# GabrielGao0310/SVT-av1_pro-anchor-v2.1.0-

Measured on AMD Instinct MI355X. Metric: CDEF+restoration+SAD Mpixels/s on 4K10b, higher is better.
Workload: dtype u16

## Files before the change

include/svtgpu.h:

```cpp
#ifndef SVTGPU_H
#define SVTGPU_H

#include <stdbool.h>
#include <stddef.h>
#include <stdint.h>

#ifdef __cplusplus
extern "C" {
#endif

#define SVTGPU_OK 0
#define SVTGPU_ERR_INVALID_ARG (-1)
#define SVTGPU_ERR_HIP (-2)
#define SVTGPU_ERR_UNSUPPORTED (-3)
#define SVTGPU_ERR_NO_DEVICE (-4)
#define SVTGPU_ERR_OOM (-5)

#define SVTGPU_BLOCK_4X4 0
#define SVTGPU_BLOCK_4X8 1
#define SVTGPU_BLOCK_8X4 2
#define SVTGPU_BLOCK_8X8 3

typedef struct SvtGpuCdefList {
    uint8_t by;
// ... 21 lines not shown
} SvtGpuConvolveParams;

#ifndef SVTGPU_CDEF_LIST_T
#define SVTGPU_CDEF_LIST_T SvtGpuCdefList
#endif
#ifndef SVTGPU_BLOCK_SIZE_T
#define SVTGPU_BLOCK_SIZE_T int32_t
#endif
#ifndef SVTGPU_SGR_PARAMS_T
#define SVTGPU_SGR_PARAMS_T SvtGpuSgrParams
#endif
#ifndef SVTGPU_CONVOLVE_PARAMS_T
#define SVTGPU_CONVOLVE_PARAMS_T SvtGpuConvolveParams
#endif
#ifndef SVTGPU_BIT_DEPTH_T
#define SVTGPU_BIT_DEPTH_T int32_t
#endif
#ifndef SVTGPU_ERROR_T
#define SVTGPU_ERROR_T uint32_t
#endif

int         svtgpu_device_available(void);
const char *svtgpu_version(void);
#define SVTGPU_ABI_VERSION 14
int32_t     svtgpu_abi_version(void);
const char *svtgpu_error_string(int code);

typedef struct SvtGpuContext SvtGpuContext;
int   svtgpu_context_create(int device, SvtGpuContext **out);
void  svtgpu_context_destroy(SvtGpuContext *ctx);
void *svtgpu_context_stream(SvtGpuContext *ctx);
int   svtgpu_synchronize(SvtGpuContext *ctx, void *stream);
int  svtgpu_stream_create(SvtGpuContext *ctx, int32_t priority, void **out_stream);
void svtgpu_stream_destroy(void *stream);
int  svtgpu_buffer_alloc(SvtGpuContext *ctx, size_t bytes, void **dev_out);
void svtgpu_buffer_free(void *dev);
int  svtgpu_buffer_upload(void *dev, const void *host, size_t bytes, void *stream);
int  svtgpu_buffer_download(void *host, const void *dev, size_t bytes, void *stream);

typedef struct SvtGpuFrame SvtGpuFrame;
int      svtgpu_frame_create(SvtGpuContext *ctx, int32_t width, int32_t height, int32_t bit_depth,
                             SvtGpuFrame **out);
void     svtgpu_frame_destroy(SvtGpuFrame *f);
int32_t  svtgpu_frame_stride(const SvtGpuFrame *f, int plane);
void    *svtgpu_frame_plane_ptr(SvtGpuFrame *f, int plane);
int svtgpu_frame_upload(SvtGpuFrame *f, int plane, const void *host, int32_t host_stride, void *stream);
int svtgpu_frame_download(const SvtGpuFrame *f, int plane, void *host, int32_t host_stride, void *stream);
// ... 725 lines not shown
int  svtgpu_lr_set_units(SvtGpuLrState *s, int32_t plane, const SvtGpuRestUnit *units, void *stream);
int  svtgpu_lr_apply_frame(SvtGpuLrState *s, const SvtGpuFrame *deblocked, const SvtGpuFrame *cdef_out,
                           SvtGpuFrame *out, const int32_t frame_type[3], void *stream);


typedef struct SvtGpuLrSearchControls {
    int32_t wn_enabled, wn_use_chroma, wn_filter_tap_lvl, wn_use_refinement, wn_max_one_refinement_step;
    int32_t sg_enabled, sg_use_chroma;
    int32_t sg_start_ep[2], sg_end_ep[2], sg_ep_inc[2], sg_refine[2];
    int32_t rdmult;
    int32_t switchable_restore_cost[3], wiener_restore_cost[2], sgrproj_restore_cost[2];
} SvtGpuLrSearchControls;
typedef struct SvtGpuLrUnitSearch {
    int64_t        sse[3];
    SvtGpuRestUnit wiener, sgrproj;
} SvtGpuLrUnitSearch;
int svtgpu_lr_search_frame(SvtGpuLrState *s, const SvtGpuFrame *recon, const SvtGpuFrame *source,
                           const SvtGpuLrSearchControls *ctrls, int32_t frame_type_out[3],
                           SvtGpuLrUnitSearch *const search_out[3], void *stream);
int svtgpu_lr_search_frame_async(SvtGpuLrState *s, const SvtGpuFrame *recon, const SvtGpuFrame *source,
                                 const SvtGpuLrSearchControls *ctrls, void *stream);
int svtgpu_lr_read_result(SvtGpuLrState *s, int32_t frame_type_out[3], void *stream);
int svtgpu_lr_read_units(SvtGpuLrState *s, int32_t plane, SvtGpuRestUnit *units_out, void *stream);
int svtgpu_lr_search_units(SvtGpuLrState *s, const SvtGpuFrame *recon, const SvtGpuFrame *source,
                           const SvtGpuLrSearchControls *ctrls, const int32_t row_begin[3], const int32_t row_end[3],
                           SvtGpuLrUnitSearch *const search_out[3], void *stream);
int svtgpu_lr_finish_plane(const SvtGpuLrSearchControls *ctrls, int32_t plane, int32_t nunits,
                           const SvtGpuLrUnitSearch *records, int32_t *frame_type_out, SvtGpuRestUnit *units_out);
int svtgpu_lr_finish_frame(const SvtGpuLrSearchControls *ctrls, const int32_t nunits[3],
                           const SvtGpuLrUnitSearch *const records[3], int32_t frame_type_out[3],
                           SvtGpuRestUnit *const units_out[3]);
int svtgpu_lr_set_tile(SvtGpuLrState *s, const int32_t units[3][4], const int32_t out[3][4], SvtGpuComm *comm);
typedef struct SvtGpuLrProfile {
    int32_t launches[6];
    float   ms[6];
    double  bytes[6];
    int32_t searches;
    float   ms_events[6];
} SvtGpuLrProfile;
int svtgpu_lr_profile(SvtGpuLrState *s, int32_t enable, SvtGpuLrProfile *totals);
int svtgpu_transfer_bytes(uint64_t *h2d, uint64_t *d2h, int32_t reset);
int svtgpu_lr_controls_for_level(int32_t wn_level, int32_t sg_level, SvtGpuLrSearchControls *c);

#define SVTGPU_CCSO_PAD 5
#define SVTGPU_CCSO_LUT 2048
typedef struct SvtGpuCcsoParams {
// ... 46 lines not shown
```

svt-av1_pro-anchor-v2.1.0-_amd/csrc/lr_common.h:

```cpp
#pragma once
#include "svtgpu_internal.h"

#include <vector>

struct SvtGpuLrState {
    SvtGpuContext  *ctx;
    int32_t         width, height;
    int32_t         unit_size[3], hunits[3], vunits[3];
    SvtGpuRestUnit *d_units[3];
    int16_t        *d_flt;
    size_t          flt_bytes;
    void           *d_work;
    size_t          work_bytes;
    void           *h_pin;
    size_t          pin_bytes;
    void           *prof;
    void                *plan_work;
    std::vector<uint8_t> plan_bytes;
    hipEvent_t           pin_free;
    hipStream_t          wst;
    hipEvent_t           ev_fork, ev_join;
    void                *d_qarena;
    size_t               qarena_bytes;
    void                *d_sxarena;
    size_t               sxarena_bytes;
    uint32_t             sx_epoch;
    int32_t              tile_units[3][4], tile_out[3][4];
    SvtGpuComm          *comm;
    int32_t             *h_fout, *h_fout_dev;
    int32_t              fin_seq, fin_pending;
    int32_t              last_ft[3];
};
void lr_profiler_destroy(void *prof);
int  lr_make_wiener_stream(SvtGpuLrState *s);
inline int lr_plane_w(const SvtGpuLrState *s, int p) { return p ? (s->width + 1) >> 1 : s->width; }
inline int lr_plane_h(const SvtGpuLrState *s, int p) { return p ? (s->height + 1) >> 1 : s->height; }
inline bool lr_frame_fits(const SvtGpuLrState *s, const SvtGpuFrame *f) {
    return f && f->width == ((s->width + 7) & ~7) && f->height == ((s->height + 7) & ~7);
}

namespace {

constexpr int NTHR = 256;
__constant__ int c_sgr_r[16][2] = {{2, 1}, {2, 1}, {2, 1}, {2, 1}, {2, 1}, {2, 1}, {2, 1}, {2, 1},
                                   {2, 1}, {2, 1}, {0, 1}, {0, 1}, {0, 1}, {0, 1}, {2, 0}, {2, 0}};
__constant__ int c_sgr_s[16][2] = {{140, 3236}, {112, 2158}, {93, 1618}, {80, 1438}, {70, 1295}, {58, 1177},
                                   {47, 1079},  {37, 996},   {30, 925},  {25, 863},  {-1, 2589}, {-1, 1618},
                                   {-1, 1177},  {-1, 925},   {56, -1},   {22, -1}};
__constant__ int c_x_by_xplus1[256] = {
    1,   128, 171, 192, 205, 213, 219, 224, 228, 230, 233, 235, 236, 238, 239, 240, 241, 242, 243, 243, 244, 244,
    245, 245, 246, 246, 247, 247, 247, 247, 248, 248, 248, 248, 249, 249, 249, 249, 249, 250, 250, 250, 250, 250,
    250, 250, 251, 251, 251, 251, 251, 251, 251, 251, 251, 251, 252, 252, 252, 252, 252, 252, 252, 252, 252, 252,
    252, 252, 252, 252, 252, 252, 252, 253, 253, 253, 253, 253, 253, 253, 253, 253, 253, 253, 253, 253, 253, 253,
    253, 253, 253, 253, 253, 253, 253, 253, 253, 253, 253, 253, 253, 253, 254, 254, 254, 254, 254, 254, 254, 254,
// ... 92 lines not shown
```

svt-av1_pro-anchor-v2.1.0-_amd/csrc/lr_search.hip:

```cpp
#include <algorithm>
#include <chrono>
#include <climits>
#include <cstdio>
#include <cstdlib>
#include <cmath>
#include <cstring>
#include <type_traits>
#include <vector>

#include "lr_common.h"


namespace {

struct Tile {
    int32_t plane, unit, x0, y0, w, h;
};
struct URect {
    int32_t h_start, h_end, v_start, v_end;
};
constexpr int PRJ_MIN0 = -96, PRJ_MAX0 = 31, PRJ_MIN1 = -32, PRJ_MAX1 = 95;
const int     kHostSgrR[16][2] = {{2, 1}, {2, 1}, {2, 1}, {2, 1}, {2, 1}, {2, 1}, {2, 1}, {2, 1},
                              {2, 1}, {2, 1}, {0, 1}, {0, 1}, {0, 1}, {0, 1}, {2, 0}, {2, 0}};
const int     kHostSgrS1[16] = {3236, 2158, 1618, 1438, 1295, 1177, 1079, 996, 925, 863, 2589, 1618, 1177, 925, -1, -1};

struct PlaneArgs {
    const void *dgd, *src;
    int16_t    *flt;
    int16_t    *dxp;
    int32_t     dstride, sstride, W, H, bd, fstride;
    int32_t     unit_base, pair_base, ne;
    int32_t     eps[16];
    int32_t     f1e[16];
    int32_t     win, nval;
    int64_t     mh_off;
};
struct SearchArgs {
    PlaneArgs      pl[3];
    const Tile    *tiles;
    const URect   *units;
    const int32_t *tile0;
};

template <typename T>
__device__ inline int px(const T *p, int stride, int W, int H, int y, int x) {
    y = min(max(y, 0), H - 1);
    x = min(max(x, 0), W - 1);
    return p[(size_t)y * stride + x];
}

__device__ inline unsigned long long wave_sum(unsigned long long v) { return wave_sum_lane63(v); }
constexpr int WAVE_LAST = 63;

constexpr int PROF_NL = 512, PROF_SP = 64;
#define PROF_BEGIN(tk)                                                                                      \
    if ((tk) && threadIdx.x == 0)                                                                           \
// ... 233 lines not shown
        }
    }
    __syncthreads();
    long long *dst = part + (size_t)tl * NVAL;
    for (int k = tid; k < NVAL; k += 256) dst[k] = out[k];
    PROF_END(tk);
}

__global__ void reduce_parts_kernel(const long long *part, const int32_t *unit_tile0, int tile_begin, int nvals,
                                    long long *out, unsigned long long *tk) {
    PROF_BEGIN(tk);
    const int u = blockIdx.x, t0 = unit_tile0[u] - tile_begin, t1 = unit_tile0[u + 1] - tile_begin;
    for (int k = blockIdx.y * blockDim.x + threadIdx.x; k < nvals; k += gridDim.y * blockDim.x) {
        long long s = 0;
        for (int t = t0; t < t1; t++) s += part[(size_t)t * nvals + k];
        out[(size_t)u * nvals + k] = s;
    }
    PROF_END(tk);
}


constexpr int SG_V = 70, SG_B = 66, SG_NT = 1024, SG_NQ = (SG_B * SG_B + SG_NT - 1) / SG_NT;
constexpr int SG_NQ2 = ((SG_B + 1) / 2 * SG_B + SG_NT - 1) / SG_NT;

__device__ inline uint32_t sgr_z(int sum, int sq, int n, int s, int sh) {
    const uint32_t a = (uint32_t)((sq + ((1 << (2 * sh)) >> 1)) >> (2 * sh));
    const uint32_t b = (uint32_t)((sum + ((1 << sh) >> 1)) >> sh);
    const uint32_t an = __umul24(a, (uint32_t)n), bb = __umul24(b, b);
    const uint32_t p  = an < bb ? 0u : an - bb;
    return min((p * (uint32_t)s + (1u << 19)) >> 20, 255u);
}
__device__ inline int sgr_ab_pack(int A, int sum, int n) {
    const int B = (int)((__umul24(__umul24((uint32_t)(256 - A), (uint32_t)sum), (uint32_t)c_one_by_x[n - 1]) + (1u << 11)) >> 12);
    return (B << 9) | A;
}

template <typename T>
__global__ __launch_bounds__(SG_NT) void sgr_flt_kernel(const SearchArgs A, unsigned long long *tk) {
    PROF_BEGIN(tk);
    __shared__ int ab1[2][SG_B * SG_B], ab2[2][SG_B * SG_B];
    __shared__ int      xby[256];
    static_assert(SG_V * SG_V * 2 <= SG_B * SG_B * 4, "tile image fits the aliased map buffer");
    uint16_t *const v = (uint16_t *)ab1[1];
    const Tile       t = A.tiles[xcd_swizzle(blockIdx.x, gridDim.x)];
    const PlaneArgs &P = A.pl[t.plane];
    const T         *d = (const T *)P.dgd;
    for (int i = threadIdx.x; i < (t.h + 6) * (t.w + 6); i += SG_NT) {
        const int r = i / (t.w + 6), c = i % (t.w + 6);
        v[r * SG_V + c] = (uint16_t)px(d, P.dstride, P.W, P.H, t.y0 + r - 3, t.x0 + c - 3);
    }
    if (threadIdx.x < 256) xby[threadIdx.x] = c_x_by_xplus1[threadIdx.x];
    __syncthreads();
    const uint16_t *v0 = v + 3 * SG_V + 3;
    auto lds_pair = [&](int a) {
        const uint32_t *w = (const uint32_t *)v + (a >> 1);
        return __builtin_amdgcn_alignbit(w[1], w[0], (a & 1) * 16);
    };
    const int       bw = t.w + 2, nq = (t.h + 2) * bw, nq2 = (t.h + 3) / 2 * bw;
    int s1[SG_NQ], q1[SG_NQ], s2[SG_NQ2], q2[SG_NQ2], m2q[SG_NQ2];
#pragma unroll
    for (int k = 0; k < SG_NQ; k++) {
        const int q = threadIdx.x + k * SG_NT;
        s1[k] = q1[k] = 0;
        if (q < nq) {
            const int y = q / bw - 1, x = q % bw - 1;
#pragma unroll
            for (int dy = -1; dy <= 1; dy++) {
                const int      a  = (y + dy + 3) * SG_V + x + 3;
                const uint32_t pr = lds_pair(a - 1);
                const int      p[3] = {(int)(pr & 0xFFFF), (int)(pr >> 16), (int)v[a + 1]};
#pragma unroll
                for (int j = 0; j < 3; j++) s1[k] += p[j], q1[k] += p[j] * p[j];
            }
        }
    }
#pragma unroll
    for (int k = 0; k < SG_NQ2; k++) {
        const int i = threadIdx.x + k * SG_NT, row = i / bw, x = i - row * bw - 1, y = 2 * row - 1;
        s2[k] = q2[k] = 0;
        m2q[k] = i < nq2 ? (y + 1) * bw + x + 1 : -1;
        if (i < nq2) {
#pragma unroll
            for (int dy = -2; dy <= 2; dy++) {
                const int      a  = (y + dy + 3) * SG_V + x + 3;
                const uint32_t pa = lds_pair(a - 2), pb = lds_pair(a);
                const int      p[5] = {(int)(pa & 0xFFFF), (int)(pa >> 16), (int)(pb & 0xFFFF), (int)(pb >> 16), (int)v[a + 2]};
#pragma unroll
                for (int j = 0; j < 5; j++) s2[k] += p[j], q2[k] += p[j] * p[j];
            }
        }
    }
    const int fr = (int)threadIdx.x / t.w, fx = (int)threadIdx.x - fr * t.w, fy0 = 4 * fr;
    const bool fon = fy0 < t.h;
    int        pix[4];
#pragma unroll
    for (int k = 0; k < 4; k++) pix[k] = fon && fy0 + k < t.h ? v0[(fy0 + k) * SG_V + fx] : 0;
    const int   fq  = fx + 1;
    const size_t fo = (size_t)(t.y0 + fy0) * P.fstride + t.x0 + fx;
    const size_t pn = (size_t)P.fstride * P.H;
    const int sh = P.bd - 8;
    auto build_ab = [&](int e) {
        const int ep = P.eps[e], r0 = c_sgr_r[ep][0], r1 = c_sgr_r[ep][1];
        int      *m1 = ab1[e & 1], *m2 = ab2[e & 1];
        if (r1 && P.f1e[e] == e) {
            const int sp = c_sgr_s[ep][1];
            uint32_t  z[SG_NQ];
            int       a[SG_NQ];
#pragma unroll
            for (int k = 0; k < SG_NQ; k++) z[k] = sgr_z(s1[k], q1[k], 9, sp, sh);
#pragma unroll
            for (int k = 0; k < SG_NQ; k++) a[k] = xby[z[k]];
#pragma unroll
            for (int k = 0; k < SG_NQ; k++) {
                const int q = threadIdx.x + k * SG_NT;
                if (q < nq) m1[q] = sgr_ab_pack(a[k], s1[k], 9);
            }
        }
        if (r0) {
            const int sp = c_sgr_s[ep][0];
            uint32_t  z[SG_NQ2];
            int       a[SG_NQ2];
#pragma unroll
            for (int k = 0; k < SG_NQ2; k++) z[k] = sgr_z(s2[k], q2[k], 25, sp, sh);
#pragma unroll
            for (int k = 0; k < SG_NQ2; k++) a[k] = xby[z[k]];
#pragma unroll
            for (int k = 0; k < SG_NQ2; k++)
                if (m2q[k] >= 0) m2[m2q[k]] = sgr_ab_pack(a[k], s2[k], 25);
        }
    };
    build_ab(0);
    __syncthreads();
    for (int e = 0; e < P.ne; e++) {
        if (e + 1 < P.ne) build_ab(e + 1);
        const int  ep = P.eps[e], r0 = c_sgr_r[ep][0], r1 = c_sgr_r[ep][1];
        const int *ab1e = ab1[e & 1], *ab2e = ab2[e & 1];
        int16_t  *f0g = P.flt + (size_t)e * 2 * pn, *f1g = f0g + pn;
        if (fon) {
            struct Row { int s, sa, c, ca; };
            auto row = [&](const int *M, int ry) {
                const int *Q = M + (min(ry, t.h) + 1) * bw + fq;
                const int  l = Q[-1], c = Q[0], r = Q[1];
                Row        w;
                w.c = c, w.ca = c & 511, w.s = l + c + r, w.sa = (l & 511) + w.ca + (r & 511);
                return w;
            };
            const int nk = min(4, t.h - fy0);
            if (r0) {
                Row up = row(ab2e, fy0 - 1);
#pragma unroll
                for (int h = 0; h < 2; h++) {
                    const int k = 2 * h;
                    if (k >= nk) break;
                    const Row dn = row(ab2e, fy0 + k + 1);
                    {
                        const int c6 = up.c + dn.c, a6 = up.ca + dn.ca;
                        const int c5 = up.s - up.c + dn.s - dn.c, a5 = up.sa - up.ca + dn.sa - dn.ca;
                        const int aa = a6 * 6 + a5 * 5, bb = ((c6 - a6) >> 9) * 6 + ((c5 - a5) >> 9) * 5;
                        f0g[fo + (size_t)k * P.fstride] =
                            (int16_t)((((int)__umul24((uint32_t)aa, (uint32_t)pix[k]) + bb + (1 << 8)) >> 9) - (pix[k] << 4));
                    }
                    if (k + 1 < nk) {
                        const int a6 = dn.ca, a5 = dn.sa - dn.ca;
                        const int aa = a6 * 6 + a5 * 5, bb = ((dn.c - a6) >> 9) * 6 + ((dn.s - dn.c - a5) >> 9) * 5;
                        f0g[fo + (size_t)(k + 1) * P.fstride] =
                            (int16_t)((((int)__umul24((uint32_t)aa, (uint32_t)pix[k + 1]) + bb + (1 << 7)) >> 8) -
                                      (pix[k + 1] << 4));
                    }
                    up = dn;
                }
            }
            if (r1 && P.f1e[e] == e) {
                Row pv = row(ab1e, fy0 - 1), cu = row(ab1e, fy0);
#pragma unroll
                for (int k = 0; k < 4; k++) {
                    if (k >= nk) break;
                    const Row nx = row(ab1e, fy0 + k + 1);
                    const int c4 = cu.s + pv.c + nx.c, a4 = cu.sa + pv.ca + nx.ca;
                    const int c3 = pv.s - pv.c + nx.s - nx.c, a3 = pv.sa - pv.ca + nx.sa - nx.ca;
                    const int aa = a4 * 4 + a3 * 3, bb = ((c4 - a4) >> 9) * 4 + ((c3 - a3) >> 9) * 3;
                    f1g[fo + (size_t)k * P.fstride] =
                        (int16_t)((((int)__umul24((uint32_t)aa, (uint32_t)pix[k]) + bb + (1 << 8)) >> 9) - (pix[k] << 4));
                    pv = cu, cu = nx;
                }
            }
        }
        __syncthreads();
    }
    PROF_END(tk);
}

typedef short v2i16s __attribute__((ext_vector_type(2)));
__device__ inline uint32_t pk_sub16(uint32_t a, uint32_t b) {
    return __builtin_bit_cast(uint32_t, __builtin_bit_cast(v2i16s, a) - __builtin_bit_cast(v2i16s, b));
}

template <typename T>
__global__ __launch_bounds__(256) void sgr_sse_kernel(const SearchArgs A, const int32_t *best, unsigned long long *err,
                                                      unsigned long long *tk) {
    PROF_BEGIN(tk);
    const Tile       t = A.tiles[xcd_swizzle(blockIdx.x, gridDim.x)];
    const PlaneArgs &P = A.pl[t.plane];
    const int       *b = best + t.unit * 4;
    const int        e = b[0], ep = b[1], xq0 = b[2], xq1 = b[3], r0 = c_sgr_r[ep][0], r1 = c_sgr_r[ep][1];
    const T         *d = (const T *)P.dgd, *s = (const T *)P.src;
    const size_t     pn = (size_t)P.fstride * P.H;
    const int16_t   *f0 = P.flt + (size_t)e * 2 * pn, *f1 = P.flt + (size_t)(e >= 0 ? P.f1e[e] : e) * 2 * pn + pn;
// ... 2233 lines not shown
        HIP_TRY(hipMalloc(&s->d_flt, 2 * flt_elems));
        s->flt_bytes = 2 * flt_elems;
    }
    uint8_t *wb = (uint8_t *)s->d_work, *hb = (uint8_t *)s->h_pin;
    auto     dp = [&](size_t o) { return (void *)(wb + o); };
    auto     hp = [&](size_t o) { return (void *)(hb + o); };
    SearchArgs A;
    std::memset(&A, 0, sizeof A);
    size_t flt_off = 0;
    for (int p = 0; p < nplanes; p++) {
        PlaneArgs &P = A.pl[p];
        P.dgd = rec->plane[p], P.src = src->plane[p], P.dstride = rec->stride[p], P.sstride = src->stride[p];
        P.W = lr_plane_w(s, p), P.H = lr_plane_h(s, p), P.bd = rec->bit_depth, P.fstride = (P.W + 63) & ~63;
        P.flt       = s->d_flt + flt_off;
        P.unit_base = pp[p].unit_base, P.pair_base = pp[p].pair_base, P.ne = pp[p].ne;
        for (int k = 0; k < pp[p].ne; k++) {
            P.eps[k] = pp[p].eps[k], P.f1e[k] = k;
            for (int j = 0; j < k; j++)
                if (kHostSgrR[P.eps[k]][1] && kHostSgrS1[P.eps[j]] == kHostSgrS1[P.eps[k]]) {
                    P.f1e[k] = j;
                    break;
                }
        }
        P.win = pp[p].win, P.nval = pp[p].nval, P.mh_off = (int64_t)pp[p].mh_off;
        P.dxp = pp[p].sg ? P.flt + (size_t)pp[p].ne * 2 * P.fstride * P.H : nullptr;
        if (pp[p].sg) flt_off += (size_t)(pp[p].ne * 2 + 1) * P.fstride * P.H;
    }
    A.tiles = (const Tile *)dp(o_tiles), A.units = (const URect *)dp(o_units), A.tile0 = (const int32_t *)dp(o_t0);
    auto *d_t0 = (int32_t *)dp(o_t0);
    LrProfiler         *prof = (LrProfiler *)s->prof;
    unsigned long long *pc   = prof ? prof->d_px : nullptr;
    auto run = [&](int c, hipStream_t ls, auto &&launch) {
        const int ev = prof ? prof->ev_begin(c, ls) : -1;
        launch(prof ? prof->slot(c) : nullptr);
        if (prof) prof->ev_end(ev, ls);
    };
    if (prof) prof->start();
    {
        uint8_t *pl = (uint8_t *)hp(h_plan);
        std::memset(pl, 0, plan_span);
        std::memcpy(pl + o_tiles, tiles.data(), sizeof(Tile) * nt_all);
        std::memcpy(pl + o_units, units.data(), sizeof(URect) * n_all);
        std::memcpy(pl + o_t0, tile0.data(), 4 * (n_all + 1));
        std::memcpy(pl + o_witem, wr_items.data(), sizeof(WrItem) * (size_t)n_wr);
        std::memcpy(pl + o_sritem, sr_items.data(), sizeof(SrItem) * (size_t)n_sr);
        std::memcpy(pl + o_dst, dst.data(), 4 * (size_t)n_all);
        if (s->plan_work != s->d_work || s->plan_bytes.size() != plan_span ||
            std::memcmp(s->plan_bytes.data(), pl, plan_span)) {
            HIP_TRY(hipMemcpyAsync(dp(0), pl, plan_span, hipMemcpyHostToDevice, st));
// ... 561 lines not shown
    }
    int32_t rb[3], re[3], cb[3], ce[3];
    for (int p = 0; p < 3; p++)
        cb[p] = s->tile_units[p][0], rb[p] = s->tile_units[p][1], ce[p] = s->tile_units[p][2], re[p] = s->tile_units[p][3];
    if (!svtgpu_comm_tiled(s->comm))
        for (int p = 0; p < 3; p++) rb[p] = cb[p] = 0, re[p] = s->vunits[p], ce[p] = s->hunits[p];
    return recon->bytes_per_sample == 2
        ? search_frame<uint16_t>(s, recon, source, ctrls, nplanes, rb, re, cb, ce, nullptr, nullptr, st, 1)
        : search_frame<uint8_t>(s, recon, source, ctrls, nplanes, rb, re, cb, ce, nullptr, nullptr, st, 1);
}

extern "C" int svtgpu_lr_read_units(SvtGpuLrState *s, int32_t plane, SvtGpuRestUnit *units_out, void *stream) {
    if (!s || plane < 0 || plane > 2 || !units_out) return SVTGPU_ERR_INVALID_ARG;
    hipStream_t st = pick_stream(s->ctx, stream);
    if (s->fin_pending)
        if (int rc = lr_collect(s, st, nullptr)) return rc;
    const size_t n = (size_t)s->hunits[plane] * s->vunits[plane];
    HIP_TRY(hipMemcpyAsync(units_out, s->d_units[plane], sizeof(SvtGpuRestUnit) * n, hipMemcpyDeviceToHost, st));
    svtgpu_count_xfer(1, sizeof(SvtGpuRestUnit) * n);
    HIP_TRY(hipStreamSynchronize(st));
    return SVTGPU_OK;
}

extern "C" int svtgpu_lr_read_result(SvtGpuLrState *s, int32_t frame_type_out[3], void *stream) {
    if (!s || !frame_type_out) return SVTGPU_ERR_INVALID_ARG;
    if (s->fin_pending) return lr_collect(s, pick_stream(s->ctx, stream), frame_type_out);
    for (int p = 0; p < 3; p++) frame_type_out[p] = s->last_ft[p];
    return SVTGPU_OK;
}
```

svt-av1_pro-anchor-v2.1.0-_amd/svtgpu.py:

```python
import ctypes
import os

import numpy as np

_HERE = os.path.dirname(os.path.abspath(__file__))
LIB_PATH = os.environ.get("SVTGPU_LIB") or os.path.join(_HERE, "lib", "libsvtgpu.so")
HEADER_PATH = os.path.join(os.path.dirname(_HERE), "include", "svtgpu.h")

SVTGPU_OK = 0
TOTAL_STRENGTHS = 64
MAX_STRENGTHS = 16


class CdefList(ctypes.Structure):
    _fields_ = [("by", ctypes.c_uint8), ("bx", ctypes.c_uint8)]


class CdefControls(ctypes.Structure):
    _fields_ = [
        ("first_pass_fs_num", ctypes.c_uint8),
        ("default_second_pass_fs_num", ctypes.c_uint8),
        ("default_first_pass_fs", ctypes.c_uint8 * TOTAL_STRENGTHS),
        ("default_second_pass_fs", ctypes.c_uint8 * TOTAL_STRENGTHS),
        ("default_first_pass_fs_uv", ctypes.c_int8 * TOTAL_STRENGTHS),
# ... 481 lines not shown
    "svtgpu_md_out_device_ptr": (_P, [_P]),
    "svtgpu_md_moments_device_ptr": (_P, [_P]),
    "svtgpu_md_expand": (ctypes.c_int, [_P, _I32, _I32, _P]),
    "svtgpu_md_layout": (None, [_P, _P, _P]),
    "svtgpu_av1_wiener_convolve_add_src": (None, [_P, ctypes.c_ssize_t, _P, ctypes.c_ssize_t, _P, _P, _I32, _I32,
                                                  ctypes.POINTER(ConvolveParams)]),
    "svtgpu_av1_highbd_wiener_convolve_add_src": (None, [_P, ctypes.c_ssize_t, _P, ctypes.c_ssize_t, _P, _P, _I32,
                                                         _I32, ctypes.POINTER(ConvolveParams), _I32]),
    "svtgpu_av1_selfguided_restoration": (None, [_P, _I32, _I32, _I32, _P, _P, _I32, _I32, _I32, _I32]),
    "svtgpu_apply_selfguided_restoration": (None, [_P, _I32, _I32, _I32, _I32, _P, _P, _I32, _P, _I32, _I32]),
    "svtgpu_lr_state_create": (ctypes.c_int, [_P, _I32, _I32, _P, ctypes.POINTER(_P)]),
    "svtgpu_lr_state_destroy": (None, [_P]),
    "svtgpu_lr_units": (ctypes.c_int, [_P, _I32, ctypes.POINTER(_I32), ctypes.POINTER(_I32)]),
    "svtgpu_lr_set_units": (ctypes.c_int, [_P, _I32, _P, _P]),
    "svtgpu_lr_apply_frame": (ctypes.c_int, [_P, _P, _P, _P, _P, _P]),
    "svtgpu_lr_search_frame": (ctypes.c_int, [_P, _P, _P, ctypes.POINTER(LrSearchControls), _P, _P, _P]),
    "svtgpu_lr_controls_for_level": (ctypes.c_int, [_I32, _I32, ctypes.POINTER(LrSearchControls)]),
    "svtgpu_lr_search_units": (ctypes.c_int, [_P, _P, _P, ctypes.POINTER(LrSearchControls), _P, _P, _P, _P]),
    "svtgpu_lr_finish_plane": (ctypes.c_int, [ctypes.POINTER(LrSearchControls), _I32, _I32, _P, _P, _P]),
    "svtgpu_lr_finish_frame": (ctypes.c_int, [ctypes.POINTER(LrSearchControls), _P, _P, _P, _P]),
    "svtgpu_lr_search_frame_async": (ctypes.c_int, [_P, _P, _P, ctypes.POINTER(LrSearchControls), _P]),
    "svtgpu_lr_read_result": (ctypes.c_int, [_P, _P, _P]),
    "svtgpu_lr_read_units": (ctypes.c_int, [_P, _I32, _P, _P]),
    "svtgpu_lr_profile": (ctypes.c_int, [_P, _I32, _P]),
    "svtgpu_transfer_bytes": (ctypes.c_int, [_P, _P, _I32]),
    "svtgpu_comm_unique_id": (ctypes.c_int, [_P]),
    "svtgpu_comm_create": (ctypes.c_int, [_P, _I32, _I32, _P, ctypes.POINTER(_P)]),
    "svtgpu_comm_create_bounded": (ctypes.c_int, [_P, _I32, _I32, _P, _I32, _I32, ctypes.POINTER(_P)]),
    "svtgpu_comm_create_host": (ctypes.c_int, [_I32, _I32, _P, ctypes.POINTER(_P)]),
    "svtgpu_comm_destroy": (None, [_P]),
    "svtgpu_comm_nranks": (_I32, [_P]),
    "svtgpu_comm_rank": (_I32, [_P]),
    "svtgpu_comm_allreduce_u64": (ctypes.c_int, [_P, _P, ctypes.c_size_t, _I32, _P]),
    "svtgpu_comm_set_timeout": (ctypes.c_int, [_P, _I32]),
    "svtgpu_comm_timeout_ms": (_I32, [_P]),
    "svtgpu_comm_set_slot": (ctypes.c_int, [_P, _I32]),
    "svtgpu_comm_failed": (_I32, [_P]),
    "svtgpu_comm_sync": (ctypes.c_int, [_P, _P]),
    "svtgpu_debug_stall": (ctypes.c_int, [_P, _P, _I32]),
    "svtgpu_shim_calls": (ctypes.c_uint64, []),
    "svtgpu_tile_plan": (ctypes.c_int, [_I32, _I32, _P, _I32, _I32, _I32, _P]),
    "svtgpu_tile_plan_sb": (ctypes.c_int, [_I32, _I32, _P, _I32, _I32, _I32, _I32, _P]),
    "svtgpu_tile_plan_crop": (ctypes.c_int, [_I32, _I32, _I32, _I32, _P, _I32, _I32, _I32, _I32, _P]),
    "svtgpu_dlf_set_tile": (ctypes.c_int, [_P, _P, _P, _P]),
    "svtgpu_dlf_set_crop": (ctypes.c_int, [_P, ctypes.c_int32, ctypes.c_int32]),
    "svtgpu_cdef_set_tile": (ctypes.c_int, [_P, _P, _P, _P]),
# ... 598 lines not shown
            check(lib().svtgpu_lr_units(h, p, ctypes.byref(hu), ctypes.byref(vu)))
            self.units.append((hu.value, vu.value))

    def set_units(self, plane, units, stream=None):
        u = np.ascontiguousarray(units, REST_UNIT_DTYPE)
        assert len(u) == self.units[plane][0] * self.units[plane][1], (len(u), self.units[plane])
        check(lib().svtgpu_lr_set_units(self.h, plane, ptr(u), stream))

    def search(self, recon, source, ctrls, stream=None, records=False):
        ft = np.zeros(3, np.int32)
        recs = [np.zeros(hu * vu, LR_UNIT_SEARCH_DTYPE) for hu, vu in self.units] if records else None
        rp = (ctypes.c_void_p * 3)(*[r.ctypes.data for r in recs]) if records else None
        check(lib().svtgpu_lr_search_frame(self.h, recon.h, source.h, ctypes.byref(ctrls), ptr(ft), rp, stream))
        return ([int(x) for x in ft], recs) if records else [int(x) for x in ft]

    def search_async(self, recon, source, ctrls, stream=None):
        check(lib().svtgpu_lr_search_frame_async(self.h, recon.h, source.h, ctypes.byref(ctrls), stream))

    def read_units(self, plane, stream=None):
        u = np.zeros(self.units[plane][0] * self.units[plane][1], REST_UNIT_DTYPE)
        check(lib().svtgpu_lr_read_units(self.h, plane, ptr(u), stream))
        return u

    def read_result(self, stream=None):
        ft = np.zeros(3, np.int32)
        check(lib().svtgpu_lr_read_result(self.h, ptr(ft), stream))
        return [int(x) for x in ft]

    def search_units(self, recon, source, ctrls, row_begin, row_end, records=None, stream=None):
        if records is None:
            records = [np.zeros(hu * vu, LR_UNIT_SEARCH_DTYPE) for hu, vu in self.units]
        rb = np.ascontiguousarray(row_begin, np.int32)
        re_ = np.ascontiguousarray(row_end, np.int32)
        rp = (ctypes.c_void_p * 3)(*[r.ctypes.data for r in records])
        check(lib().svtgpu_lr_search_units(self.h, recon.h, source.h, ctypes.byref(ctrls), ptr(rb), ptr(re_), rp,
                                           stream))
        return records

    PROFILE_CLASSES = ("stats", "sgr_filters", "wiener_trials", "projection", "other", "sgr_moments")

    def profile(self, enable=True, events=False, serial=False):
        if enable is True:
            mask = -1
        elif not enable:
            mask = 0
        else:
# ... 11 lines not shown
        out["searches"] = int(raw["searches"][0])
        return out

    def set_tile(self, units=None, out=None, comm=None):
        check(lib().svtgpu_lr_set_tile(self.h, _rects3(units), _rects3(out), comm.h if comm else None))

    def apply(self, deblocked, cdef_out, out, frame_type, stream=None):
        ft = None if frame_type is None else np.ascontiguousarray(frame_type, np.int32)
        check(lib().svtgpu_lr_apply_frame(self.h, deblocked.h, cdef_out.h, out.h, None if ft is None else ptr(ft),
                                          stream))

    def close(self):
        if self.h:
            lib().svtgpu_lr_state_destroy(self.h)
            self.h = None

    def __del__(self):
        try:
            self.close()
        except Exception:
            pass


def lr_controls(wn_level, sg_level, rdmult=0, switchable=(0, 0, 0), wiener=(0, 0), sgrproj=(0, 0)):
    c = LrSearchControls()
    check(lib().svtgpu_lr_controls_for_level(wn_level, sg_level, ctypes.byref(c)))
    c.rdmult = rdmult
    for i, v in enumerate(switchable):
        c.switchable_restore_cost[i] = v
    for i, v in enumerate(wiener):
        c.wiener_restore_cost[i] = v
    for i, v in enumerate(sgrproj):
        c.sgrproj_restore_cost[i] = v
    return c


def lr_finish_plane(ctrls, plane, records):
    r = np.ascontiguousarray(records, LR_UNIT_SEARCH_DTYPE)
    units = np.zeros(len(r), REST_UNIT_DTYPE)
    ft = _I32()
    check(lib().svtgpu_lr_finish_plane(ctypes.byref(ctrls), plane, len(r), ptr(r), ctypes.byref(ft), ptr(units)))
    return ft.value, units


def lr_finish_frame(ctrls, records):
    rs = [np.ascontiguousarray(r, LR_UNIT_SEARCH_DTYPE) for r in records]
# ... 260 lines not shown
```

Baseline: 3547.

## Restructure SGR filter kernel: precompute variance terms, repack A/B maps, 2x2 output per thread

The self-guided filter search kernel now turns the box sums into variance terms once, before the eps loop, and pre-multiplies sums by the one_by_x constants. The strength values per eps are resolved on the host, so the hot loop no longer does constant-memory radius/strength lookups. The A/B map packing is reformulated to store 256-A with an 11-bit field so each output pixel needs fewer ops. Each thread now produces a 2x2 pixel block with paired 32-bit stores instead of a 4-row column, and a waves-per-EU hint is added. A debug readback API for the SGR filter planes is also added, which slightly enlarges the state struct and bumps the ABI version.

```diff
diff --git a/include/svtgpu.h b/include/svtgpu.h
--- a/include/svtgpu.h
+++ b/include/svtgpu.h
@@ -67,7 +67,7 @@
 
 int         svtgpu_device_available(void);
 const char *svtgpu_version(void);
-#define SVTGPU_ABI_VERSION 14
+#define SVTGPU_ABI_VERSION 15
 int32_t     svtgpu_abi_version(void);
 const char *svtgpu_error_string(int code);
 
@@ -839,6 +839,8 @@
                                  const SvtGpuLrSearchControls *ctrls, void *stream);
 int svtgpu_lr_read_result(SvtGpuLrState *s, int32_t frame_type_out[3], void *stream);
 int svtgpu_lr_read_units(SvtGpuLrState *s, int32_t plane, SvtGpuRestUnit *units_out, void *stream);
+int svtgpu_lr_read_sgr_planes(SvtGpuLrState *s, int32_t plane, int32_t slot, int32_t *ep_out, int16_t *flt0,
+                              int16_t *flt1, void *stream);
 int svtgpu_lr_search_units(SvtGpuLrState *s, const SvtGpuFrame *recon, const SvtGpuFrame *source,
                            const SvtGpuLrSearchControls *ctrls, const int32_t row_begin[3], const int32_t row_end[3],
                            SvtGpuLrUnitSearch *const search_out[3], void *stream);
diff --git a/svt-av1_pro-anchor-v2.1.0-_amd/csrc/lr_common.h b/svt-av1_pro-anchor-v2.1.0-_amd/csrc/lr_common.h
--- a/svt-av1_pro-anchor-v2.1.0-_amd/csrc/lr_common.h
+++ b/svt-av1_pro-anchor-v2.1.0-_amd/csrc/lr_common.h
@@ -30,6 +30,8 @@
     int32_t             *h_fout, *h_fout_dev;
     int32_t              fin_seq, fin_pending;
     int32_t              last_ft[3];
+    int16_t             *sg_flt[3];
+    int32_t              sg_fstride[3], sg_w[3], sg_h[3], sg_ne[3], sg_eps[3][16], sg_f1e[3][16];
 };
 void lr_profiler_destroy(void *prof);
 int  lr_make_wiener_stream(SvtGpuLrState *s);
diff --git a/svt-av1_pro-anchor-v2.1.0-_amd/csrc/lr_search.hip b/svt-av1_pro-anchor-v2.1.0-_amd/csrc/lr_search.hip
--- a/svt-av1_pro-anchor-v2.1.0-_amd/csrc/lr_search.hip
+++ b/svt-av1_pro-anchor-v2.1.0-_amd/csrc/lr_search.hip
@@ -23,6 +23,7 @@
 const int     kHostSgrR[16][2] = {{2, 1}, {2, 1}, {2, 1}, {2, 1}, {2, 1}, {2, 1}, {2, 1}, {2, 1},
                               {2, 1}, {2, 1}, {0, 1}, {0, 1}, {0, 1}, {0, 1}, {2, 0}, {2, 0}};
 const int     kHostSgrS1[16] = {3236, 2158, 1618, 1438, 1295, 1177, 1079, 996, 925, 863, 2589, 1618, 1177, 925, -1, -1};
+const int     kHostSgrS0[16] = {140, 112, 93, 80, 70, 58, 47, 37, 30, 25, -1, -1, -1, -1, 56, 22};
 
 struct PlaneArgs {
     const void *dgd, *src;
@@ -32,6 +33,7 @@
     int32_t     unit_base, pair_base, ne;
     int32_t     eps[16];
     int32_t     f1e[16];
+    int32_t     es0[16], es1[16];
     int32_t     win, nval;
     int64_t     mh_off;
 };
@@ -311,24 +313,33 @@
 
 constexpr int SG_V = 70, SG_B = 66, SG_NT = 1024, SG_NQ = (SG_B * SG_B + SG_NT - 1) / SG_NT;
 constexpr int SG_NQ2 = ((SG_B + 1) / 2 * SG_B + SG_NT - 1) / SG_NT;
-
-__device__ inline uint32_t sgr_z(int sum, int sq, int n, int s, int sh) {
+constexpr int      SG_AB = 11;
+constexpr uint32_t SG_AM = (1u << SG_AB) - 1;
+
+__device__ inline uint32_t sgr_p(int sum, int sq, int n, int sh) {
     const uint32_t a = (uint32_t)((sq + ((1 << (2 * sh)) >> 1)) >> (2 * sh));
     const uint32_t b = (uint32_t)((sum + ((1 << sh) >> 1)) >> sh);
     const uint32_t an = __umul24(a, (uint32_t)n), bb = __umul24(b, b);
-    const uint32_t p  = an < bb ? 0u : an - bb;
-    return min((p * (uint32_t)s + (1u << 19)) >> 20, 255u);
-}
-__device__ inline int sgr_ab_pack(int A, int sum, int n) {
-    const int B = (int)((__umul24(__umul24((uint32_t)(256 - A), (uint32_t)sum), (uint32_t)c_one_by_x[n - 1]) + (1u << 11)) >> 12);
-    return (B << 9) | A;
+    return an < bb ? 0u : an - bb;
+}
+__device__ inline uint32_t sgr_z(uint32_t p, int s) { return min((p * (uint32_t)s + (1u << 19)) >> 20, 255u); }
+__device__ inline int sgr_ab_pack(int Am, uint32_t so) {
+    const uint32_t x = __umul24((uint32_t)Am, so) + (1u << 11);
+    return (int)(((x >> 1) & ~SG_AM) | (uint32_t)Am);
+}
+template <int WA, int WB, int SH>
+__device__ inline int sgr_pixel(uint32_t ca, uint32_t cb, int npix) {
+    const int ma = __mul24((int)(ca & SG_AM), npix) + (int)(ca >> SG_AB);
+    const int mb = __mul24((int)(cb & SG_AM), npix) + (int)(cb >> SG_AB);
+    return (__mul24(ma, WA) + (__mul24(mb, WB) + (1 << (SH - 1)))) >> SH;
 }
 
 template <typename T>
-__global__ __launch_bounds__(SG_NT) void sgr_flt_kernel(const SearchArgs A, unsigned long long *tk) {
+__global__ __launch_bounds__(SG_NT) __attribute__((amdgpu_waves_per_eu(8))) void sgr_flt_kernel(const SearchArgs A,
+                                                                                                unsigned long long *tk) {
     PROF_BEGIN(tk);
     __shared__ int ab1[2][SG_B * SG_B], ab2[2][SG_B * SG_B];
-    __shared__ int      xby[256];
+    __shared__ int xby[256];
     static_assert(SG_V * SG_V * 2 <= SG_B * SG_B * 4, "tile image fits the aliased map buffer");
     uint16_t *const v = (uint16_t *)ab1[1];
     const Tile       t = A.tiles[xcd_swizzle(blockIdx.x, gridDim.x)];
@@ -338,7 +349,7 @@
         const int r = i / (t.w + 6), c = i % (t.w + 6);
         v[r * SG_V + c] = (uint16_t)px(d, P.dstride, P.W, P.H, t.y0 + r - 3, t.x0 + c - 3);
     }
-    if (threadIdx.x < 256) xby[threadIdx.x] = c_x_by_xplus1[threadIdx.x];
+    if (threadIdx.x < 256) xby[threadIdx.x] = 256 - c_x_by_xplus1[threadIdx.x];
     __syncthreads();
     const uint16_t *v0 = v + 3 * SG_V + 3;
     auto lds_pair = [&](int a) {
@@ -347,6 +358,7 @@
     };
     const int       bw = t.w + 2, nq = (t.h + 2) * bw, nq2 = (t.h + 3) / 2 * bw;
     int s1[SG_NQ], q1[SG_NQ], s2[SG_NQ2], q2[SG_NQ2], m2q[SG_NQ2];
+    const int sh = P.bd - 8;
 #pragma unroll
     for (int k = 0; k < SG_NQ; k++) {
         const int q = threadIdx.x + k * SG_NT;
@@ -362,6 +374,7 @@
                 for (int j = 0; j < 3; j++) s1[k] += p[j], q1[k] += p[j] * p[j];
             }
         }
+        q1[k] = (int)sgr_p(s1[k], q1[k], 9, sh), s1[k] = (int)__umul24((uint32_t)s1[k], 455u);
     }
 #pragma unroll
     for (int k = 0; k < SG_NQ2; k++) {
@@ -378,100 +391,96 @@
                 for (int j = 0; j < 5; j++) s2[k] += p[j], q2[k] += p[j] * p[j];
             }
         }
-    }
-    const int fr = (int)threadIdx.x / t.w, fx = (int)threadIdx.x - fr * t.w, fy0 = 4 * fr;
-    const bool fon = fy0 < t.h;
-    int        pix[4];
-#pragma unroll
-    for (int k = 0; k < 4; k++) pix[k] = fon && fy0 + k < t.h ? v0[(fy0 + k) * SG_V + fx] : 0;
-    const int   fq  = fx + 1;
-    const size_t fo = (size_t)(t.y0 + fy0) * P.fstride + t.x0 + fx;
-    const size_t pn = (size_t)P.fstride * P.H;
-    const int sh = P.bd - 8;
+        q2[k] = (int)sgr_p(s2[k], q2[k], 25, sh), s2[k] = (int)__umul24((uint32_t)s2[k], 164u);
+    }
+    const int  cpn = (t.w + 1) >> 1, fr = (int)threadIdx.x / cpn;
+    const bool fon = 2 * fr < t.h;
+    const int  fx = fon ? 2 * ((int)threadIdx.x - fr * cpn) : 0, fy0 = fon ? 2 * fr : 0;
+    const bool row1 = fy0 + 1 < t.h, col1 = fx + 1 < t.w;
+    int        npix[2][2];
+#pragma unroll
+    for (int j = 0; j < 2; j++)
+#pragma unroll
+        for (int i = 0; i < 2; i++) npix[j][i] = -(int)v0[(fy0 + j) * SG_V + fx + i];
+    int mrow[4];
+#pragma unroll
+    for (int j = 0; j < 4; j++) mrow[j] = (min(fy0 - 1 + j, t.h) + 1) * bw + fx;
+    const uint32_t fob = 2u * ((uint32_t)(t.y0 + fy0) * (uint32_t)P.fstride + (uint32_t)(t.x0 + fx));
+    const size_t   pn  = (size_t)P.fstride * P.H;
     auto build_ab = [&](int e) {
-        const int ep = P.eps[e], r0 = c_sgr_r[ep][0], r1 = c_sgr_r[ep][1];
+        const int sp0 = P.es0[e], sp1 = P.es1[e];
         int      *m1 = ab1[e & 1], *m2 = ab2[e & 1];
-        if (r1 && P.f1e[e] == e) {
-            const int sp = c_sgr_s[ep][1];
-            uint32_t  z[SG_NQ];
-            int       a[SG_NQ];
-#pragma unroll
-            for (int k = 0; k < SG_NQ; k++) z[k] = sgr_z(s1[k], q1[k], 9, sp, sh);
+        if (sp1) {
+            uint32_t z[SG_NQ];
+            int      a[SG_NQ];
+#pragma unroll
+            for (int k = 0; k < SG_NQ; k++) z[k] = sgr_z((uint32_t)q1[k], sp1);
 #pragma unroll
             for (int k = 0; k < SG_NQ; k++) a[k] = xby[z[k]];
 #pragma unroll
             for (int k = 0; k < SG_NQ; k++) {
                 const int q = threadIdx.x + k * SG_NT;
-                if (q < nq) m1[q] = sgr_ab_pack(a[k], s1[k], 9);
-            }
-        }
-        if (r0) {
-            const int sp = c_sgr_s[ep][0];
-            uint32_t  z[SG_NQ2];
-            int       a[SG_NQ2];
-#pragma unroll
-            for (int k = 0; k < SG_NQ2; k++) z[k] = sgr_z(s2[k], q2[k], 25, sp, sh);
+                if (q < nq) m1[q] = sgr_ab_pack(a[k], (uint32_t)s1[k]);
+            }
+        }
+        if (sp0) {
+            uint32_t z[SG_NQ2];
+            int      a[SG_NQ2];
+#pragma unroll
+            for (int k = 0; k < SG_NQ2; k++) z[k] = sgr_z((uint32_t)q2[k], sp0);
 #pragma unroll
             for (int k = 0; k < SG_NQ2; k++) a[k] = xby[z[k]];
 #pragma unroll
             for (int k = 0; k < SG_NQ2; k++)
-                if (m2q[k] >= 0) m2[m2q[k]] = sgr_ab_pack(a[k], s2[k], 25);
-        }
+                if (m2q[k] >= 0) m2[m2q[k]] = sgr_ab_pack(a[k], (uint32_t)s2[k]);
+        }
+    };
+    struct Row { uint32_t s[2], c[2]; };
+    auto row = [&](const int *M, int j) {
+        const int     *Q  = M + mrow[j];
+        const uint32_t w0 = (uint32_t)Q[0], w1 = (uint32_t)Q[1], w2 = (uint32_t)Q[2], w3 = (uint32_t)Q[3];
+        Row            w;
+        w.c[0] = w1, w.c[1] = w2, w.s[0] = w0 + w1 + w2, w.s[1] = w1 + w2 + w3;
+        return w;
+    };
+    auto store2 = [&](int16_t *plane_row, int g0, int g1) {
+        char *a = (char *)plane_row + fob;
+        if (col1)
+            *(uint32_t *)a = pack2(g0, g1);
+        else
+            *(int16_t *)a = (int16_t)g0;
     };
     build_ab(0);
     __syncthreads();
     for (int e = 0; e < P.ne; e++) {
         if (e + 1 < P.ne) build_ab(e + 1);
-        const int  ep = P.eps[e], r0 = c_sgr_r[ep][0], r1 = c_sgr_r[ep][1];
+        const int  sp0 = P.es0[e], sp1 = P.es1[e];
         const int *ab1e = ab1[e & 1], *ab2e = ab2[e & 1];
-        int16_t  *f0g = P.flt + (size_t)e * 2 * pn, *f1g = f0g + pn;
+        int16_t   *f0g = P.flt + (size_t)e * 2 * pn, *f1g = f0g + pn;
         if (fon) {
-            struct Row { int s, sa, c, ca; };
-            auto row = [&](const int *M, int ry) {
-                const int *Q = M + (min(ry, t.h) + 1) * bw + fq;
-                const int  l = Q[-1], c = Q[0], r = Q[1];
-                Row        w;
-                w.c = c, w.ca = c & 511, w.s = l + c + r, w.sa = (l & 511) + w.ca + (r & 511);
-                return w;
-            };
-            const int nk = min(4, t.h - fy0);
-            if (r0) {
-                Row up = row(ab2e, fy0 - 1);
-#pragma unroll
-                for (int h = 0; h < 2; h++) {
-                    const int k = 2 * h;
-                    if (k >= nk) break;
-                    const Row dn = row(ab2e, fy0 + k + 1);
-                    {
-                        const int c6 = up.c + dn.c, a6 = up.ca + dn.ca;
-                        const int c5 = up.s - up.c + dn.s - dn.c, a5 = up.sa - up.ca + dn.sa - dn.ca;
-                        const int aa = a6 * 6 + a5 * 5, bb = ((c6 - a6) >> 9) * 6 + ((c5 - a5) >> 9) * 5;
-                        f0g[fo + (size_t)k * P.fstride] =
-                            (int16_t)((((int)__umul24((uint32_t)aa, (uint32_t)pix[k]) + bb + (1 << 8)) >> 9) - (pix[k] << 4));
-                    }
-                    if (k + 1 < nk) {
-                        const int a6 = dn.ca, a5 = dn.sa - dn.ca;
-                        const int aa = a6 * 6 + a5 * 5, bb = ((dn.c - a6) >> 9) * 6 + ((dn.s - dn.c - a5) >> 9) * 5;
-                        f0g[fo + (size_t)(k + 1) * P.fstride] =
-                            (int16_t)((((int)__umul24((uint32_t)aa, (uint32_t)pix[k + 1]) + bb + (1 << 7)) >> 8) -
-                                      (pix[k + 1] << 4));
-                    }
-                    up = dn;
+            if (sp0) {
+                const Row up = row(ab2e, 0), dn = row(ab2e, 2);
+                int       g[2][2];
+#pragma unroll
+                for (int i = 0; i < 2; i++) {
+                    const uint32_t c6 = up.c[i] + dn.c[i], c5 = up.s[i] + dn.s[i] - c6;
+                    g[0][i] = sgr_pixel<6, 5, 9>(c6, c5, npix[0][i]);
+                    g[1][i] = sgr_pixel<6, 5, 8>(dn.c[i], dn.s[i] - dn.c[i], npix[1][i]);
                 }
-            }
-            if (r1 && P.f1e[e] == e) {
-                Row pv = row(ab1e, fy0 - 1), cu = row(ab1e, fy0);
-#pragma unroll
-                for (int k = 0; k < 4; k++) {
-                    if (k >= nk) break;
-                    const Row nx = row(ab1e, fy0 + k + 1);
-                    const int c4 = cu.s + pv.c + nx.c, a4 = cu.sa + pv.ca + nx.ca;
-                    const int c3 = pv.s - pv.c + nx.s - nx.c, a3 = pv.sa - pv.ca + nx.sa - nx.ca;
-                    const int aa = a4 * 4 + a3 * 3, bb = ((c4 - a4) >> 9) * 4 + ((c3 - a3) >> 9) * 3;
-                    f1g[fo + (size_t)k * P.fstride] =
-                        (int16_t)((((int)__umul24((uint32_t)aa, (uint32_t)pix[k]) + bb + (1 << 8)) >> 9) - (pix[k] << 4));
-                    pv = cu, cu = nx;
+                store2(f0g, g[0][0], g[0][1]);
+                if (row1) store2(f0g + P.fstride, g[1][0], g[1][1]);
+            }
+            if (sp1) {
+                const Row r0 = row(ab1e, 0), r1 = row(ab1e, 1), r2 = row(ab1e, 2), r3 = row(ab1e, 3);
+                int       g[2][2];
+#pragma unroll
+                for (int i = 0; i < 2; i++) {
+                    const uint32_t cn0 = r0.c[i] + r2.c[i], cn1 = r1.c[i] + r3.c[i];
+                    g[0][i] = sgr_pixel<4, 3, 9>(r1.s[i] + cn0, r0.s[i] + r2.s[i] - cn0, npix[0][i]);
+                    g[1][i] = sgr_pixel<4, 3, 9>(r2.s[i] + cn1, r1.s[i] + r3.s[i] - cn1, npix[1][i]);
                 }
+                store2(f1g, g[0][0], g[0][1]);
+                if (row1) store2(f1g + P.fstride, g[1][0], g[1][1]);
             }
         }
         __syncthreads();
@@ -2751,9 +2760,19 @@
                     break;
                 }
         }
+        for (int k = 0; k < pp[p].ne; k++) {
+            P.es0[k] = kHostSgrR[P.eps[k]][0] ? kHostSgrS0[P.eps[k]] : 0;
+            P.es1[k] = kHostSgrR[P.eps[k]][1] && P.f1e[k] == k ? kHostSgrS1[P.eps[k]] : 0;
+        }
         P.win = pp[p].win, P.nval = pp[p].nval, P.mh_off = (int64_t)pp[p].mh_off;
         P.dxp = pp[p].sg ? P.flt + (size_t)pp[p].ne * 2 * P.fstride * P.H : nullptr;
         if (pp[p].sg) flt_off += (size_t)(pp[p].ne * 2 + 1) * P.fstride * P.H;
+    }
+    for (int p = 0; p < 3; p++) {
+        const bool sg = p < nplanes && pp[p].sg;
+        s->sg_flt[p] = sg ? A.pl[p].flt : nullptr, s->sg_ne[p] = sg ? A.pl[p].ne : 0;
+        s->sg_fstride[p] = A.pl[p].fstride, s->sg_w[p] = A.pl[p].W, s->sg_h[p] = A.pl[p].H;
+        for (int k = 0; k < 16; k++) s->sg_eps[p][k] = A.pl[p].eps[k], s->sg_f1e[p][k] = A.pl[p].f1e[k];
     }
     A.tiles = (const Tile *)dp(o_tiles), A.units = (const URect *)dp(o_units), A.tile0 = (const int32_t *)dp(o_t0);
     auto *d_t0 = (int32_t *)dp(o_t0);
@@ -3361,6 +3380,26 @@
     return SVTGPU_OK;
 }
 
+extern "C" int svtgpu_lr_read_sgr_planes(SvtGpuLrState *s, int32_t plane, int32_t slot, int32_t *ep_out, int16_t *flt0,
+                                        int16_t *flt1, void *stream) {
+    if (!s || plane < 0 || plane > 2 || !ep_out || !flt0 || !flt1) return SVTGPU_ERR_INVALID_ARG;
+    if (!s->sg_flt[plane] || slot < 0 || slot >= s->sg_ne[plane]) return SVTGPU_ERR_INVALID_ARG;
+    hipStream_t st = pick_stream(s->ctx, stream);
+    if (s->fin_pending)
+        if (int rc = lr_collect(s, st, nullptr)) return rc;
+    const int    ep = s->sg_eps[plane][slot], W = s->sg_w[plane], H = s->sg_h[plane], fs = s->sg_fstride[plane];
+    const size_t pn = (size_t)fs * H;
+    *ep_out = ep;
+    if (kHostSgrR[ep][0])
+        HIP_TRY(hipMemcpy2DAsync(flt0, 2 * (size_t)W, s->sg_flt[plane] + (size_t)slot * 2 * pn, 2 * (size_t)fs, 2 * (size_t)W,
+                                 H, hipMemcpyDeviceToHost, st));
+    if (kHostSgrR[ep][1])
+        HIP_TRY(hipMemcpy2DAsync(flt1, 2 * (size_t)W, s->sg_flt[plane] + (size_t)s->sg_f1e[plane][slot] * 2 * pn + pn,
+                                 2 * (size_t)fs, 2 * (size_t)W, H, hipMemcpyDeviceToHost, st));
+    HIP_TRY(hipStreamSynchronize(st));
+    return SVTGPU_OK;
+}
+
 extern "C" int svtgpu_lr_read_result(SvtGpuLrState *s, int32_t frame_type_out[3], void *stream) {
     if (!s || !frame_type_out) return SVTGPU_ERR_INVALID_ARG;
     if (s->fin_pending) return lr_collect(s, pick_stream(s->ctx, stream), frame_type_out);
diff --git a/svt-av1_pro-anchor-v2.1.0-_amd/svtgpu.py b/svt-av1_pro-anchor-v2.1.0-_amd/svtgpu.py
--- a/svt-av1_pro-anchor-v2.1.0-_amd/svtgpu.py
+++ b/svt-av1_pro-anchor-v2.1.0-_amd/svtgpu.py
@@ -527,6 +527,7 @@
     "svtgpu_lr_search_frame_async": (ctypes.c_int, [_P, _P, _P, ctypes.POINTER(LrSearchControls), _P]),
     "svtgpu_lr_read_result": (ctypes.c_int, [_P, _P, _P]),
     "svtgpu_lr_read_units": (ctypes.c_int, [_P, _I32, _P, _P]),
+    "svtgpu_lr_read_sgr_planes": (ctypes.c_int, [_P, _I32, _I32, ctypes.POINTER(_I32), _P, _P, _P]),
     "svtgpu_lr_profile": (ctypes.c_int, [_P, _I32, _P]),
     "svtgpu_transfer_bytes": (ctypes.c_int, [_P, _P, _I32]),
     "svtgpu_comm_unique_id": (ctypes.c_int, [_P]),
@@ -1171,6 +1172,14 @@
         check(lib().svtgpu_lr_read_units(self.h, plane, ptr(u), stream))
         return u
 
+    def read_sgr_planes(self, plane, slot, stream=None):
+        w = (self.width + 1) >> 1 if plane else self.width
+        h = (self.height + 1) >> 1 if plane else self.height
+        f0, f1, ep = np.zeros((h, w), np.int16), np.zeros((h, w), np.int16), _I32()
+        check(lib().svtgpu_lr_read_sgr_planes(self.h, plane, slot, ctypes.byref(ep), ptr(f0), ptr(f1), stream))
+        r0, r1 = SGR_RADII[ep.value]
+        return ep.value, f0 if r0 else None, f1 if r1 else None
+
     def read_result(self, stream=None):
         ft = np.zeros(3, np.int32)
         check(lib().svtgpu_lr_read_result(self.h, ptr(ft), stream))
@@ -1228,6 +1237,9 @@
             pass
 
 
+SGR_RADII = [(2, 1)] * 10 + [(0, 1)] * 4 + [(2, 0)] * 2
+
+
 def lr_controls(wn_level, sg_level, rdmult=0, switchable=(0, 0, 0), wiener=(0, 0), sgrproj=(0, 0)):
     c = LrSearchControls()
     check(lib().svtgpu_lr_controls_for_level(wn_level, sg_level, ctypes.byref(c)))
```

New measurement: 3674 (median of 6 runs). 1.04x the previous value.
